# NVlabs/gbrl

Hardware: AMD Instinct MI355X
Metric: trees-fit/sec + predict rows/sec at batch=2^20, feat=128, depth=6, out=8 (higher is better)
Workload: dtype int32 fixed-point sums / f32 scores

## Files before the change

gbrl_amd/csrc/quantile.hip:

```cpp
#include "kernels.h"
#include "hooks.h"
#include "kernels_common.h"
#include "small_prep.h"

#include <algorithm>
#include <cstdint>
#include <cstdlib>

namespace gbrl {
namespace kern {

namespace {

constexpr int kMaxSplit = 4095;
constexpr int kClasses = 2 * (kMaxSplit + 1);

__global__ __launch_bounds__(256) void k_transpose_keys(const float *__restrict__ obs, int n, int F, uint32_t *__restrict__ kt) {
    __shared__ uint32_t tile[64][65];
    const int r0 = blockIdx.x * 64, f0 = blockIdx.y * 64;
    const int tx = threadIdx.x & 63, ty = threadIdx.x >> 6;
    for (int i = ty; i < 64; i += 4) {
        const int r = r0 + i, f = f0 + tx;
        tile[i][tx] = (r < n && f < F) ? float_to_key(obs[static_cast<size_t>(r) * F + f]) : 0xffffffffu;
    }
    __syncthreads();
    for (int i = ty; i < 64; i += 4) {
        const int f = f0 + i, r = r0 + tx;
        if (f < F && r < n) kt[static_cast<size_t>(f) * n + r] = tile[tx][i];
    }
}

__global__ __launch_bounds__(256) void k_transpose_keys_v4(const float *__restrict__ obs, int n, int F, uint32_t *__restrict__ kt) {
    __shared__ uint32_t tile[64][65];
    const int r0 = blockIdx.x * 64, f0 = blockIdx.y * 64;
    const int q = threadIdx.x & 15, p = threadIdx.x >> 4;
    float4 v[4];
#pragma unroll
    for (int i = 0; i < 4; ++i) {
        const int r = r0 + i * 16 + p, f = f0 + 4 * q;
        v[i] = (r < n && f < F) ? *reinterpret_cast<const float4 *>(obs + static_cast<size_t>(r) * F + f) : make_float4(0.f, 0.f, 0.f, 0.f);
    }
#pragma unroll
    for (int i = 0; i < 4; ++i) {
        uint32_t *t = &tile[i * 16 + p][4 * q];
        t[0] = float_to_key(v[i].x); t[1] = float_to_key(v[i].y); t[2] = float_to_key(v[i].z); t[3] = float_to_key(v[i].w);
    }
    __syncthreads();
#pragma unroll
    for (int i = 0; i < 4; ++i) {
        const int f = f0 + i * 16 + p, r = r0 + 4 * q;
        if (f < F && r < n) {
            const uint4 o = make_uint4(tile[4 * q][i * 16 + p], tile[4 * q + 1][i * 16 + p], tile[4 * q + 2][i * 16 + p], tile[4 * q + 3][i * 16 + p]);
            *reinterpret_cast<uint4 *>(kt + static_cast<size_t>(f) * n + r) = o;
        }
    }
}

__global__ __launch_bounds__(1024) void k_sample_splitters(const uint32_t *__restrict__ kt, int n, int S, int n_split,
                                                           uint32_t *__restrict__ splitters, uint32_t *__restrict__ splitters_bfs,
                                                           uint32_t *__restrict__ sample_out ) {
    extern __shared__ uint32_t s[];
    const int f = blockIdx.x;
    const uint32_t *col = kt + static_cast<size_t>(f) * n;
    if (n <= S) {
        for (int i = threadIdx.x; i < S; i += blockDim.x) s[i] = i < n ? col[i] : 0xffffffffu;
    } else {
        const double stride = static_cast<double>(n) / S;
        for (int i = threadIdx.x; i < S; i += blockDim.x) {
            const long long lo = static_cast<long long>(i * stride), hi = static_cast<long long>((i + 1) * stride);
            uint32_t h = (static_cast<uint32_t>(i) * 2654435761u) ^ (static_cast<uint32_t>(f) * 40503u + 0x9e3779b9u);
            h ^= h >> 15; h *= 2246822519u; h ^= h >> 13;
            const long long span = hi > lo ? hi - lo : 1;
            long long idx = lo + static_cast<long long>(h % static_cast<uint32_t>(span));
            if (idx >= n) idx = n - 1;
            s[i] = col[idx];
        }
    }
    __syncthreads();
    if (sample_out) {
        for (int i = threadIdx.x; i < S; i += blockDim.x) sample_out[static_cast<size_t>(f) * S + i] = s[i];
        return;
    }
    for (int k = 2; k <= S; k <<= 1) {
        for (int j = k >> 1; j > 0; j >>= 1) {
            for (int i = threadIdx.x; i < S; i += blockDim.x) {
                const int ixj = i ^ j;
                if (ixj > i) {
                    const uint32_t a = s[i], b = s[ixj];
                    const bool up = (i & k) == 0;
                    if ((a > b) == up) { s[i] = b; s[ixj] = a; }
                }
            }
            __syncthreads();
        }
    }
    const int step = S / (n_split + 1);
    for (int j = threadIdx.x; j < n_split; j += blockDim.x) splitters[static_cast<size_t>(f) * kMaxSplit + j] = s[(j + 1) * step - 1];
    int levels = 0;
    while ((1 << levels) < n_split + 1) ++levels;
    for (int i = threadIdx.x; i < n_split; i += blockDim.x) {
        const int L = 31 - __clz(i + 1), pp = i + 1 - (1 << L);
        const int q = ((2 * pp + 1) << (levels - 1 - L)) - 1;
        splitters_bfs[static_cast<size_t>(f) * kMaxSplit + i] = s[(q + 1) * step - 1];
    }
}

__global__ __launch_bounds__(1024) void k_sort_quantiles(const uint32_t *__restrict__ kt, int n, int S, const int64_t *__restrict__ cum, int B,
                                                         uint32_t *__restrict__ thr_keys, float *__restrict__ thr_floats, int F,
                                                         uint16_t *__restrict__ codes) {
    extern __shared__ uint32_t s[];
    sort_quantiles_body<false>(kt, n, S, cum, B, thr_keys, thr_floats, F, static_cast<int>(blockIdx.x), codes, s);
}

__global__ __launch_bounds__(1024) void k_union_splitters(const int64_t *__restrict__ uni, int SU, int n_split,
                                                          uint32_t *__restrict__ splitters, uint32_t *__restrict__ splitters_bfs) {
    extern __shared__ uint32_t s[];
    const int f = blockIdx.x;
    for (int i = threadIdx.x; i < SU; i += blockDim.x) s[i] = static_cast<uint32_t>(uni[static_cast<size_t>(f) * SU + i]);
    __syncthreads();
    for (int k = 2; k <= SU; k <<= 1) {
        for (int j = k >> 1; j > 0; j >>= 1) {
            for (int i = threadIdx.x; i < SU; i += blockDim.x) {
                const int ixj = i ^ j;
                if (ixj > i) {
                    const uint32_t a = s[i], b = s[ixj];
                    const bool up = (i & k) == 0;
                    if ((a > b) == up) { s[i] = b; s[ixj] = a; }
                }
            }
            __syncthreads();
        }
    }
    const int step = SU / (n_split + 1);
    for (int j = threadIdx.x; j < n_split; j += blockDim.x) splitters[static_cast<size_t>(f) * kMaxSplit + j] = s[(j + 1) * step - 1];
    int levels = 0;
    while ((1 << levels) < n_split + 1) ++levels;
    for (int i = threadIdx.x; i < n_split; i += blockDim.x) {
        const int L = 31 - __clz(i + 1), pp = i + 1 - (1 << L);
        const int q = ((2 * pp + 1) << (levels - 1 - L)) - 1;
        splitters_bfs[static_cast<size_t>(f) * kMaxSplit + i] = s[(q + 1) * step - 1];
    }
}
__global__ void k_place_sample(const uint32_t *__restrict__ samp, int F, int S, int rank, int SU, int64_t *__restrict__ uni) {
    const size_t i = static_cast<size_t>(blockIdx.x) * blockDim.x + threadIdx.x;
    if (i >= static_cast<size_t>(F) * S) return;
    const size_t f = i / S, j = i % S;
    uni[f * SU + static_cast<size_t>(rank) * S + j] = samp[i];
}
__global__ void k_counts_to_i64(const uint32_t *__restrict__ partial, int n_chunks, size_t fc, int64_t *__restrict__ out) {
    const size_t i = static_cast<size_t>(blockIdx.x) * blockDim.x + threadIdx.x;
    if (i >= fc) return;
    int64_t v = 0;
    for (int q = 0; q < n_chunks; ++q) v += partial[static_cast<size_t>(q) * fc + i];
    out[i] = v;
}
__global__ __launch_bounds__(256) void k_select_count(const uint32_t *__restrict__ lists, const uint32_t *__restrict__ tgt_off,
                                                      const uint32_t *__restrict__ tgt_len, const uint32_t *__restrict__ prefix,
                                                      int bit, int n_targets, int64_t *__restrict__ counts) {
    const int t = blockIdx.x * (blockDim.x / kWave) + (threadIdx.x / kWave);
    const int lane = threadIdx.x & (kWave - 1);
    if (t >= n_targets) return;
    const uint32_t off = tgt_off[t];
    uint32_t c = 0;
    if (off < 0xfffffffeu) {
        const uint32_t trial = prefix[t] | (1u << bit);
        const uint32_t *keys = lists + off;
        const uint32_t m = tgt_len[t];
        for (uint32_t i = lane; i < m; i += kWave) c += keys[i] < trial ? 1u : 0u;
        for (int o = kWave / 2; o > 0; o >>= 1) c += __shfl_xor(c, o, kWave);
    }
    if (lane == 0) counts[t] = c;
}
__global__ void k_select_update(uint32_t *__restrict__ prefix, const int64_t *__restrict__ counts, const uint32_t *__restrict__ tgt_off,
                                const uint32_t *__restrict__ tgt_rank, int bit, int n_targets, uint32_t *__restrict__ thr_keys) {
    const int t = blockIdx.x * blockDim.x + threadIdx.x;
    if (t >= n_targets) return;
    if (tgt_off[t] >= 0xfffffffeu) return;
    uint32_t p = prefix[t];
    if (counts[t] < static_cast<int64_t>(tgt_rank[t])) p |= (1u << bit);
    prefix[t] = p;
    if (bit == 0) thr_keys[t] = p;
}

__device__ __forceinline__ int classify(const uint32_t *e, int levels, uint32_t key) {
    int i = 0;
    uint32_t last_ge = 0;
    bool went_left = false;
    for (int l = 0; l < levels; ++l) {
        const uint32_t v = e[i];
        const bool lt = v < key;
        if (!lt) { last_ge = v; went_left = true; }
        i = 2 * i + 1 + (lt ? 1 : 0);
    }
    const int j = i - ((1 << levels) - 1);
    return 2 * j + ((went_left && last_ge == key) ? 1 : 0);
}
constexpr int KQ = 8;
__device__ __forceinline__ void classifyN(const uint32_t *e, int levels, const uint32_t (&key)[KQ], int (&cls)[KQ]) {
    int i[KQ];
    uint32_t ge[KQ];
    bool wl[KQ];
#pragma unroll
    for (int q = 0; q < KQ; ++q) { i[q] = 0; ge[q] = 0; wl[q] = false; }
    for (int l = 0; l < levels; ++l) {
#pragma unroll
        for (int q = 0; q < KQ; ++q) {
            const uint32_t v = e[i[q]];
            const bool lt = v < key[q];
            if (!lt) { ge[q] = v; wl[q] = true; }
            i[q] = 2 * i[q] + 1 + (lt ? 1 : 0);
        }
    }
#pragma unroll
    for (int q = 0; q < KQ; ++q) cls[q] = 2 * (i[q] - ((1 << levels) - 1)) + ((wl[q] && ge[q] == key[q]) ? 1 : 0);
}

constexpr int kCountThreads = 512;
__global__ __launch_bounds__(kCountThreads) void k_class_count(const uint32_t *__restrict__ kt, int n, int n_split,
                                                               const uint32_t *__restrict__ splitters, int chunk,
                                                               uint32_t *__restrict__ partial ) {
    __shared__ uint32_t sp[kMaxSplit + 1];
    __shared__ uint32_t cnt[kClasses];
    const int f = blockIdx.y;
    for (int i = threadIdx.x; i < n_split; i += kCountThreads) sp[i] = splitters[static_cast<size_t>(f) * kMaxSplit + i];
    for (int i = threadIdx.x; i < kClasses; i += kCountThreads) cnt[i] = 0;
    __syncthreads();
    const uint32_t *col = kt + static_cast<size_t>(f) * n;
    const int lo = blockIdx.x * chunk, hi = min(n, lo + chunk);
    int levels = 0;
    while ((1 << levels) < n_split + 1) ++levels;
    int i = lo + threadIdx.x;
    for (; i + (KQ - 1) * kCountThreads < hi; i += KQ * kCountThreads) {
        uint32_t k[KQ];
#pragma unroll
        for (int q = 0; q < KQ; ++q) k[q] = col[i + q * kCountThreads];
        int cls[KQ];
        classifyN(sp, levels, k, cls);
#pragma unroll
        for (int q = 0; q < KQ; ++q) atomicAdd(&cnt[cls[q]], 1u);
    }
    for (; i < hi; i += kCountThreads) atomicAdd(&cnt[classify(sp, levels, col[i])], 1u);
    __syncthreads();
    uint32_t *dst = partial + (static_cast<size_t>(blockIdx.x) * gridDim.y + f) * kClasses;
    for (int c = threadIdx.x; c < kClasses; c += kCountThreads) dst[c] = cnt[c];
}

__global__ __launch_bounds__(1024) void k_targets(const uint32_t *__restrict__ partial, int n_chunks, int F,
                                                  const int64_t *__restrict__ global_counts ,
                                                  const uint32_t *__restrict__ splitters, const int64_t *__restrict__ cum, int B,
                                                  uint32_t *__restrict__ class_off ,
                                                  uint32_t *__restrict__ tgt_off ,
                                                  uint32_t *__restrict__ tgt_len, uint32_t *__restrict__ tgt_rank,
                                                  uint32_t *__restrict__ thr_keys ,
                                                  uint32_t *__restrict__ alloc , uint32_t max_elems,
                                                  uint32_t *__restrict__ overflow) {
    __shared__ uint32_t pre[kClasses];
    __shared__ int32_t tcls[1024];
    const int f = blockIdx.x;
    uint32_t *coff = class_off + static_cast<size_t>(f) * kClasses;
    __shared__ uint32_t loc_cnt[kClasses];
    for (int c = threadIdx.x; c < kClasses; c += blockDim.x) {
        uint32_t v = 0;
        for (int q = 0; q < n_chunks; ++q) v += partial[(static_cast<size_t>(q) * F + f) * kClasses + c];
        loc_cnt[c] = v;
        pre[c] = global_counts ? static_cast<uint32_t>(global_counts[static_cast<size_t>(f) * kClasses + c]) : v;
    }
    __syncthreads();
    {
        const int base = threadIdx.x * 8;
        uint32_t loc[8], run = 0;
        for (int q = 0; q < 8; ++q) { run += pre[base + q]; loc[q] = run; }
        __shared__ uint32_t tot[1024];
        tot[threadIdx.x] = run;
        __syncthreads();
        for (int o = 1; o < 1024; o <<= 1) {
            const uint32_t v = threadIdx.x >= o ? tot[threadIdx.x - o] : 0;
            __syncthreads();
            tot[threadIdx.x] += v;
            __syncthreads();
        }
        const uint32_t off = threadIdx.x ? tot[threadIdx.x - 1] : 0;
        for (int q = 0; q < 8; ++q) pre[base + q] = loc[q] + off;
        __syncthreads();
    }
    for (int k0 = 0; k0 < B; k0 += 1024) {
        const int k = k0 + threadIdx.x;
        int c = -1;
        uint32_t want = 0, before = 0;
        if (k < B) {
            want = static_cast<uint32_t>(cum[k]);
            int lo = 0, hi = kClasses - 1;
            while (lo < hi) {
                const int mid = (lo + hi) >> 1;
                if (pre[mid] < want) lo = mid + 1; else hi = mid;
            }
            c = lo;
            before = c ? pre[c - 1] : 0;
        }
        tcls[threadIdx.x] = c;
        __syncthreads();
        if (k < B) {
            const size_t t = static_cast<size_t>(f) * B + k;
            tgt_rank[t] = want - before;
            if (c & 1) {
                thr_keys[t] = splitters[static_cast<size_t>(f) * kMaxSplit + (c >> 1)];
                tgt_off[t] = 0xffffffffu;
                tgt_len[t] = 0;
            } else {
                const bool first = (threadIdx.x == 0) ? (coff[c] == 0xffffffffu) : (tcls[threadIdx.x - 1] != c);
                const uint32_t len = loc_cnt[c];
                if (first) {
                    const uint32_t off = atomicAdd(&alloc[0], len);
                    if (off + len > max_elems || off + len < off) { atomicExch(overflow, 1u); coff[c] = 0xfffffffeu; }
                    else coff[c] = off;
                }
                tgt_len[t] = len;
            }
        }
        __syncthreads();
        if (k < B && !(c & 1)) tgt_off[static_cast<size_t>(f) * B + k] = coff[c];
        __syncthreads();
    }
}

__global__ __launch_bounds__(kCountThreads) void k_extract(const uint32_t *__restrict__ kt, int n, int n_split,
                                                           const uint32_t *__restrict__ splitters, int chunk,
                                                           const uint32_t *__restrict__ class_off,
                                                           const uint32_t *__restrict__ partial, uint32_t *__restrict__ out) {
    __shared__ uint32_t sp[kMaxSplit + 1];
    __shared__ uint32_t cur[kClasses];
    const int f = blockIdx.y, F = gridDim.y;
    for (int i = threadIdx.x; i < n_split; i += kCountThreads) sp[i] = splitters[static_cast<size_t>(f) * kMaxSplit + i];
    {
        constexpr int PER = kClasses / kCountThreads;
        uint32_t off[PER];
#pragma unroll
        for (int u = 0; u < PER; ++u) off[u] = class_off[static_cast<size_t>(f) * kClasses + threadIdx.x + u * kCountThreads];
        for (unsigned q = 0; q < blockIdx.x; ++q) {
            uint32_t add[PER];
#pragma unroll
            for (int u = 0; u < PER; ++u) add[u] = partial[(static_cast<size_t>(q) * F + f) * kClasses + threadIdx.x + u * kCountThreads];
#pragma unroll
            for (int u = 0; u < PER; ++u) off[u] += add[u];
        }
#pragma unroll
        for (int u = 0; u < PER; ++u) {
            const uint32_t base = class_off[static_cast<size_t>(f) * kClasses + threadIdx.x + u * kCountThreads];
            cur[threadIdx.x + u * kCountThreads] = base < 0xfffffffeu ? off[u] : 0xffffffffu;
        }
    }
    __syncthreads();
    const uint32_t *col = kt + static_cast<size_t>(f) * n;
    const int lo = blockIdx.x * chunk, hi = min(n, lo + chunk);
    int levels = 0;
    while ((1 << levels) < n_split + 1) ++levels;
    int i = lo + threadIdx.x;
    for (; i + (KQ - 1) * kCountThreads < hi; i += KQ * kCountThreads) {
        uint32_t k[KQ];
#pragma unroll
        for (int q = 0; q < KQ; ++q) k[q] = col[i + q * kCountThreads];
        int cls[KQ];
        classifyN(sp, levels, k, cls);
#pragma unroll
        for (int q = 0; q < KQ; ++q)
            if (cur[cls[q]] != 0xffffffffu) out[atomicAdd(&cur[cls[q]], 1u)] = k[q];
    }
    for (; i < hi; i += kCountThreads) {
        const uint32_t key = col[i];
        const int cls = classify(sp, levels, key);
        if (cur[cls] != 0xffffffffu) out[atomicAdd(&cur[cls], 1u)] = key;
    }
}

__global__ __launch_bounds__(256) void k_select(const uint32_t *__restrict__ lists, const uint32_t *__restrict__ tgt_off,
                                                const uint32_t *__restrict__ tgt_len, const uint32_t *__restrict__ tgt_rank,
                                                int n_targets, uint32_t *__restrict__ thr_keys) {
    const int t = blockIdx.x * (blockDim.x / kWave) + (threadIdx.x / kWave);
    const int lane = threadIdx.x & (kWave - 1);
    if (t >= n_targets) return;
    const uint32_t off = tgt_off[t];
    if (off >= 0xfffffffeu) return;
    const uint32_t *keys = lists + off;
    const uint32_t m = tgt_len[t], r = tgt_rank[t];
    uint32_t p = 0;
    constexpr int R = 16;
    if (m <= kWave * R) {
        uint32_t k[R];
#pragma unroll
        for (int q = 0; q < R; ++q) k[q] = (lane + q * kWave) < m ? keys[lane + q * kWave] : 0xffffffffu;
        for (int bit = 31; bit >= 0; --bit) {
            const uint32_t trial = p | (1u << bit);
            uint32_t c = 0;
#pragma unroll
            for (int q = 0; q < R; ++q) c += k[q] < trial ? 1u : 0u;
            for (int o = kWave / 2; o > 0; o >>= 1) c += __shfl_xor(c, o, kWave);
            if (c < r) p = trial;
        }
    } else {
        for (int bit = 31; bit >= 0; --bit) {
            const uint32_t trial = p | (1u << bit);
            uint32_t c = 0;
            for (uint32_t i = lane; i < m; i += kWave) c += keys[i] < trial ? 1u : 0u;
            for (int o = kWave / 2; o > 0; o >>= 1) c += __shfl_xor(c, o, kWave);
            if (c < r) p = trial;
        }
    }
    if (lane == 0) thr_keys[t] = p;
}

constexpr int kGroup = 16;
constexpr int kBinTiles = 16;
__global__ __launch_bounds__(256) void k_bin_cols(const uint32_t *__restrict__ kt, int n, int F, const uint32_t *__restrict__ thr,
                                                  int B, int levels, int tiles_per_block, uint16_t *__restrict__ codes) {
    extern __shared__ uint32_t lds[];
    const int P = (1 << levels) - 1;
    uint32_t *t = lds;
    uint16_t *tile_buf = reinterpret_cast<uint16_t *>(lds + kGroup * P);
    const int g = blockIdx.y;
    for (int i = threadIdx.x; i < kGroup * P; i += 256) {
        const int fl = i / P, e = i % P, f = g * kGroup + fl;
        const int L = 31 - __clz(e + 1), pp = e + 1 - (1 << L);
        const int q = ((2 * pp + 1) << (levels - 1 - L)) - 1;
        t[i] = (f < F && q < B) ? thr[static_cast<size_t>(f) * B + q] : 0xffffffffu;
    }
    __syncthreads();
    for (int tile = 0; tile < tiles_per_block; ++tile) {
        const int r0 = (blockIdx.x * tiles_per_block + tile) * 256;
        if (r0 >= n) break;
        const int r = r0 + threadIdx.x;
        const int rr = r < n ? r : n - 1;
        uint32_t key[kGroup];
#pragma unroll
        for (int q = 0; q < kGroup; ++q) {
            const int f = g * kGroup + q;
            key[q] = kt[static_cast<size_t>(f < F ? f : F - 1) * n + rr];
        }
#pragma unroll
        for (int fl0 = 0; fl0 < kGroup; fl0 += 8) {
            int idx[8];
#pragma unroll
            for (int q = 0; q < 8; ++q) idx[q] = 0;
            for (int l = 0; l < levels; ++l) {
#pragma unroll
                for (int q = 0; q < 8; ++q) idx[q] = 2 * idx[q] + 1 + ((t[(fl0 + q) * P + idx[q]] < key[fl0 + q]) ? 1 : 0);
            }
#pragma unroll
            for (int q = 0; q < 8; ++q) {
                const int f = g * kGroup + fl0 + q;
                int code = idx[q] - P;
                if (code > B) code = B;
                tile_buf[threadIdx.x * kGroup + fl0 + q] = static_cast<uint16_t>((f < F && r < n) ? code : 0);
            }
        }
        __syncthreads();
        const int rows = min(256, n - r0);
        {
            uint4 *dst = reinterpret_cast<uint4 *>(codes + (static_cast<size_t>(g) * n + r0) * kGroup);
            const uint4 *src = reinterpret_cast<const uint4 *>(tile_buf);
            for (int i = threadIdx.x; i < rows * 2; i += 256) dst[i] = src[i];
        }
        __syncthreads();
    }
}

#define GBRL_BIN_STEP_L8_F0(U, T, K) \
    asm volatile("v_lshl_add_u32 %8, %0, 2, %24\n ds_read_b32 %8, %8 offset:0\n" \
                 "v_lshl_add_u32 %9, %1, 2, %24\n ds_read_b32 %9, %9 offset:1024\n" \
                 "v_lshl_add_u32 %10, %2, 2, %24\n ds_read_b32 %10, %10 offset:2048\n" \
                 "v_lshl_add_u32 %11, %3, 2, %24\n ds_read_b32 %11, %11 offset:3072\n" \
                 "v_lshl_add_u32 %12, %4, 2, %24\n ds_read_b32 %12, %12 offset:4096\n" \
                 "v_lshl_add_u32 %13, %5, 2, %24\n ds_read_b32 %13, %13 offset:5120\n" \
                 "v_lshl_add_u32 %14, %6, 2, %24\n ds_read_b32 %14, %14 offset:6144\n" \
                 "v_lshl_add_u32 %15, %7, 2, %24\n ds_read_b32 %15, %15 offset:7168\n" \
                 "s_waitcnt lgkmcnt(0)\n" \
                 "v_cmp_lt_u32 vcc, %8, %16\n v_addc_co_u32 %0, vcc, %0, %0, vcc\n" \
                 "v_cmp_lt_u32 vcc, %9, %17\n v_addc_co_u32 %1, vcc, %1, %1, vcc\n" \
                 "v_cmp_lt_u32 vcc, %10, %18\n v_addc_co_u32 %2, vcc, %2, %2, vcc\n" \
                 "v_cmp_lt_u32 vcc, %11, %19\n v_addc_co_u32 %3, vcc, %3, %3, vcc\n" \
                 "v_cmp_lt_u32 vcc, %12, %20\n v_addc_co_u32 %4, vcc, %4, %4, vcc\n" \
                 "v_cmp_lt_u32 vcc, %13, %21\n v_addc_co_u32 %5, vcc, %5, %5, vcc\n" \
                 "v_cmp_lt_u32 vcc, %14, %22\n v_addc_co_u32 %6, vcc, %6, %6, vcc\n" \
                 "v_cmp_lt_u32 vcc, %15, %23\n v_addc_co_u32 %7, vcc, %7, %7, vcc\n" \
                 : "+v"(U[0]), "+v"(U[1]), "+v"(U[2]), "+v"(U[3]), "+v"(U[4]), "+v"(U[5]), "+v"(U[6]), "+v"(U[7]), \
                   "=&v"(T[0]), "=&v"(T[1]), "=&v"(T[2]), "=&v"(T[3]), "=&v"(T[4]), "=&v"(T[5]), "=&v"(T[6]), "=&v"(T[7]) \
                 : "v"(K[0]), "v"(K[1]), "v"(K[2]), "v"(K[3]), "v"(K[4]), "v"(K[5]), "v"(K[6]), "v"(K[7]), "s"(lds_base) \
                 : "vcc", "memory")
#define GBRL_BIN_STEP_L8_F8(U, T, K) \
    asm volatile("v_lshl_add_u32 %8, %0, 2, %24\n ds_read_b32 %8, %8 offset:8192\n" \
                 "v_lshl_add_u32 %9, %1, 2, %24\n ds_read_b32 %9, %9 offset:9216\n" \
                 "v_lshl_add_u32 %10, %2, 2, %24\n ds_read_b32 %10, %10 offset:10240\n" \
                 "v_lshl_add_u32 %11, %3, 2, %24\n ds_read_b32 %11, %11 offset:11264\n" \
                 "v_lshl_add_u32 %12, %4, 2, %24\n ds_read_b32 %12, %12 offset:12288\n" \
                 "v_lshl_add_u32 %13, %5, 2, %24\n ds_read_b32 %13, %13 offset:13312\n" \
                 "v_lshl_add_u32 %14, %6, 2, %24\n ds_read_b32 %14, %14 offset:14336\n" \
                 "v_lshl_add_u32 %15, %7, 2, %24\n ds_read_b32 %15, %15 offset:15360\n" \
                 "s_waitcnt lgkmcnt(0)\n" \
                 "v_cmp_lt_u32 vcc, %8, %16\n v_addc_co_u32 %0, vcc, %0, %0, vcc\n" \
                 "v_cmp_lt_u32 vcc, %9, %17\n v_addc_co_u32 %1, vcc, %1, %1, vcc\n" \
                 "v_cmp_lt_u32 vcc, %10, %18\n v_addc_co_u32 %2, vcc, %2, %2, vcc\n" \
                 "v_cmp_lt_u32 vcc, %11, %19\n v_addc_co_u32 %3, vcc, %3, %3, vcc\n" \
                 "v_cmp_lt_u32 vcc, %12, %20\n v_addc_co_u32 %4, vcc, %4, %4, vcc\n" \
                 "v_cmp_lt_u32 vcc, %13, %21\n v_addc_co_u32 %5, vcc, %5, %5, vcc\n" \
                 "v_cmp_lt_u32 vcc, %14, %22\n v_addc_co_u32 %6, vcc, %6, %6, vcc\n" \
                 "v_cmp_lt_u32 vcc, %15, %23\n v_addc_co_u32 %7, vcc, %7, %7, vcc\n" \
                 : "+v"(U[0]), "+v"(U[1]), "+v"(U[2]), "+v"(U[3]), "+v"(U[4]), "+v"(U[5]), "+v"(U[6]), "+v"(U[7]), \
                   "=&v"(T[0]), "=&v"(T[1]), "=&v"(T[2]), "=&v"(T[3]), "=&v"(T[4]), "=&v"(T[5]), "=&v"(T[6]), "=&v"(T[7]) \
                 : "v"(K[0]), "v"(K[1]), "v"(K[2]), "v"(K[3]), "v"(K[4]), "v"(K[5]), "v"(K[6]), "v"(K[7]), "s"(lds_base) \
                 : "vcc", "memory")
#define GBRL_BIN_STEP_L9_F0(U, T, K) \
    asm volatile("v_lshl_add_u32 %8, %0, 2, %24\n ds_read_b32 %8, %8 offset:0\n" \
                 "v_lshl_add_u32 %9, %1, 2, %24\n ds_read_b32 %9, %9 offset:2048\n" \
                 "v_lshl_add_u32 %10, %2, 2, %24\n ds_read_b32 %10, %10 offset:4096\n" \
                 "v_lshl_add_u32 %11, %3, 2, %24\n ds_read_b32 %11, %11 offset:6144\n" \
                 "v_lshl_add_u32 %12, %4, 2, %24\n ds_read_b32 %12, %12 offset:8192\n" \
                 "v_lshl_add_u32 %13, %5, 2, %24\n ds_read_b32 %13, %13 offset:10240\n" \
                 "v_lshl_add_u32 %14, %6, 2, %24\n ds_read_b32 %14, %14 offset:12288\n" \
                 "v_lshl_add_u32 %15, %7, 2, %24\n ds_read_b32 %15, %15 offset:14336\n" \
                 "s_waitcnt lgkmcnt(0)\n" \
                 "v_cmp_lt_u32 vcc, %8, %16\n v_addc_co_u32 %0, vcc, %0, %0, vcc\n" \
                 "v_cmp_lt_u32 vcc, %9, %17\n v_addc_co_u32 %1, vcc, %1, %1, vcc\n" \
                 "v_cmp_lt_u32 vcc, %10, %18\n v_addc_co_u32 %2, vcc, %2, %2, vcc\n" \
                 "v_cmp_lt_u32 vcc, %11, %19\n v_addc_co_u32 %3, vcc, %3, %3, vcc\n" \
                 "v_cmp_lt_u32 vcc, %12, %20\n v_addc_co_u32 %4, vcc, %4, %4, vcc\n" \
                 "v_cmp_lt_u32 vcc, %13, %21\n v_addc_co_u32 %5, vcc, %5, %5, vcc\n" \
                 "v_cmp_lt_u32 vcc, %14, %22\n v_addc_co_u32 %6, vcc, %6, %6, vcc\n" \
                 "v_cmp_lt_u32 vcc, %15, %23\n v_addc_co_u32 %7, vcc, %7, %7, vcc\n" \
                 : "+v"(U[0]), "+v"(U[1]), "+v"(U[2]), "+v"(U[3]), "+v"(U[4]), "+v"(U[5]), "+v"(U[6]), "+v"(U[7]), \
                   "=&v"(T[0]), "=&v"(T[1]), "=&v"(T[2]), "=&v"(T[3]), "=&v"(T[4]), "=&v"(T[5]), "=&v"(T[6]), "=&v"(T[7]) \
                 : "v"(K[0]), "v"(K[1]), "v"(K[2]), "v"(K[3]), "v"(K[4]), "v"(K[5]), "v"(K[6]), "v"(K[7]), "s"(lds_base) \
                 : "vcc", "memory")
#define GBRL_BIN_STEP_L9_F8(U, T, K) \
    asm volatile("v_lshl_add_u32 %8, %0, 2, %24\n ds_read_b32 %8, %8 offset:16384\n" \
                 "v_lshl_add_u32 %9, %1, 2, %24\n ds_read_b32 %9, %9 offset:18432\n" \
                 "v_lshl_add_u32 %10, %2, 2, %24\n ds_read_b32 %10, %10 offset:20480\n" \
                 "v_lshl_add_u32 %11, %3, 2, %24\n ds_read_b32 %11, %11 offset:22528\n" \
                 "v_lshl_add_u32 %12, %4, 2, %24\n ds_read_b32 %12, %12 offset:24576\n" \
                 "v_lshl_add_u32 %13, %5, 2, %24\n ds_read_b32 %13, %13 offset:26624\n" \
                 "v_lshl_add_u32 %14, %6, 2, %24\n ds_read_b32 %14, %14 offset:28672\n" \
                 "v_lshl_add_u32 %15, %7, 2, %24\n ds_read_b32 %15, %15 offset:30720\n" \
                 "s_waitcnt lgkmcnt(0)\n" \
                 "v_cmp_lt_u32 vcc, %8, %16\n v_addc_co_u32 %0, vcc, %0, %0, vcc\n" \
                 "v_cmp_lt_u32 vcc, %9, %17\n v_addc_co_u32 %1, vcc, %1, %1, vcc\n" \
                 "v_cmp_lt_u32 vcc, %10, %18\n v_addc_co_u32 %2, vcc, %2, %2, vcc\n" \
                 "v_cmp_lt_u32 vcc, %11, %19\n v_addc_co_u32 %3, vcc, %3, %3, vcc\n" \
                 "v_cmp_lt_u32 vcc, %12, %20\n v_addc_co_u32 %4, vcc, %4, %4, vcc\n" \
                 "v_cmp_lt_u32 vcc, %13, %21\n v_addc_co_u32 %5, vcc, %5, %5, vcc\n" \
                 "v_cmp_lt_u32 vcc, %14, %22\n v_addc_co_u32 %6, vcc, %6, %6, vcc\n" \
                 "v_cmp_lt_u32 vcc, %15, %23\n v_addc_co_u32 %7, vcc, %7, %7, vcc\n" \
                 : "+v"(U[0]), "+v"(U[1]), "+v"(U[2]), "+v"(U[3]), "+v"(U[4]), "+v"(U[5]), "+v"(U[6]), "+v"(U[7]), \
                   "=&v"(T[0]), "=&v"(T[1]), "=&v"(T[2]), "=&v"(T[3]), "=&v"(T[4]), "=&v"(T[5]), "=&v"(T[6]), "=&v"(T[7]) \
                 : "v"(K[0]), "v"(K[1]), "v"(K[2]), "v"(K[3]), "v"(K[4]), "v"(K[5]), "v"(K[6]), "v"(K[7]), "s"(lds_base) \
                 : "vcc", "memory")

template <int LEVELS>
__global__ __launch_bounds__(256) void k_bin_cols_fast(const uint32_t *__restrict__ kt, int n, int F, const uint32_t *__restrict__ thr,
                                                       int B, int tiles_per_block, uint16_t *__restrict__ codes) {
    constexpr int S = 1 << LEVELS;
    extern __shared__ uint32_t lds[];
    uint32_t *t = lds;
    uint32_t *tile_buf = lds + kGroup * S;
    const uint32_t lds_base = static_cast<uint32_t>(reinterpret_cast<uintptr_t>(t));
    const int g = blockIdx.y;
    for (int i = threadIdx.x; i < kGroup * S; i += 256) {
        const int fl = i >> LEVELS, u = i & (S - 1), f = g * kGroup + fl;
        uint32_t v = 0xffffffffu;
        if (u > 0) {
            const int L = 31 - __clz(u), pp = u - (1 << L);
            const int q = ((2 * pp + 1) << (LEVELS - 1 - L)) - 1;
            if (f < F && q < B) v = thr[static_cast<size_t>(f) * B + q];
        }
        t[i] = v;
    }
    __syncthreads();
    for (int tile = 0; tile < tiles_per_block; ++tile) {
        const int r0 = (blockIdx.x * tiles_per_block + tile) * 256;
        if (r0 >= n) break;
        const int r = r0 + threadIdx.x;
        const int rr = r < n ? r : n - 1;
        uint32_t key[kGroup];
#pragma unroll
        for (int q = 0; q < kGroup; ++q) {
            const int f = g * kGroup + q;
            key[q] = kt[static_cast<size_t>(f < F ? f : F - 1) * n + rr];
        }
        uint32_t word[kGroup / 2];
#pragma unroll
        for (int half = 0; half < 2; ++half) {
            uint32_t u[8], tv[8], kk[8];
#pragma unroll
            for (int q = 0; q < 8; ++q) { u[q] = 1; kk[q] = key[half * 8 + q]; }
#pragma unroll
            for (int l = 0; l < LEVELS; ++l) {
                if constexpr (LEVELS == 8) { if (half == 0) { GBRL_BIN_STEP_L8_F0(u, tv, kk); } else { GBRL_BIN_STEP_L8_F8(u, tv, kk); } }
                else                       { if (half == 0) { GBRL_BIN_STEP_L9_F0(u, tv, kk); } else { GBRL_BIN_STEP_L9_F8(u, tv, kk); } }
            }
#pragma unroll
            for (int q = 0; q < 8; q += 2) {
                const int f0 = g * kGroup + half * 8 + q;
                uint32_t c0 = min(u[q] - S, static_cast<uint32_t>(B)), c1 = min(u[q + 1] - S, static_cast<uint32_t>(B));
                if (!(f0 < F && r < n)) c0 = 0;
                if (!(f0 + 1 < F && r < n)) c1 = 0;
                word[half * 4 + q / 2] = c0 | (c1 << 16);
            }
        }
        uint4 *row = reinterpret_cast<uint4 *>(tile_buf + threadIdx.x * 8);
        row[0] = make_uint4(word[0], word[1], word[2], word[3]);
        row[1] = make_uint4(word[4], word[5], word[6], word[7]);
        __syncthreads();
        const int rows = min(256, n - r0);
        {
            uint4 *dst = reinterpret_cast<uint4 *>(codes + (static_cast<size_t>(g) * n + r0) * kGroup);
            const uint4 *src = reinterpret_cast<const uint4 *>(tile_buf);
            for (int i = threadIdx.x; i < rows * 2; i += 256) dst[i] = src[i];
        }
        __syncthreads();
    }
}
#undef GBRL_BIN_STEP_L8_F0
#undef GBRL_BIN_STEP_L8_F8
#undef GBRL_BIN_STEP_L9_F0
#undef GBRL_BIN_STEP_L9_F8

__global__ void k_scatter_cat_codes_grouped(const uint16_t *__restrict__ cat_codes, int n, int Fc, int F,
                                            uint16_t *__restrict__ codes) {
    const size_t i = static_cast<size_t>(blockIdx.x) * blockDim.x + threadIdx.x;
    if (i >= static_cast<size_t>(n) * Fc) return;
    const size_t r = i / Fc;
    const int slot = F + static_cast<int>(i % Fc);
    codes[(static_cast<size_t>(slot / kGroup) * n + r) * kGroup + (slot % kGroup)] = cat_codes[i];
}

}

void transpose_keys(const float *obs, int n, int F, uint32_t *kt, hipStream_t s) {
    dim3 grid((n + 63) / 64, (F + 63) / 64);
    const bool plain = [] { const char *e = hooks::raw(hooks::TRANSPOSE_PLAIN); return e && e[0] == '1'; }();
    if ((F & 3) == 0 && (n & 3) == 0 && !plain && (reinterpret_cast<uintptr_t>(obs) & 15) == 0 && (reinterpret_cast<uintptr_t>(kt) & 15) == 0)
        hipLaunchKernelGGL(k_transpose_keys_v4, grid, dim3(256), 0, s, obs, n, F, kt);
    else
        hipLaunchKernelGGL(k_transpose_keys, grid, dim3(256), 0, s, obs, n, F, kt);
}

QuantilePlan quantile_plan(int n) {
    QuantilePlan p;
    int S = 64;
    while (S < n && S < 4096) S <<= 1;
    p.sample = S;
    p.n_split = S - 1 < kMaxSplit ? S - 1 : kMaxSplit;
    p.n_chunks = n >= (1 << 18) ? 8 : (n >= (1 << 15) ? 2 : 1);
    p.chunk = (n + p.n_chunks - 1) / p.n_chunks;
    return p;
}

void sample_splitters(const uint32_t *kt, int n, int F, const QuantilePlan &p, uint32_t *splitters, uint32_t *splitters_bfs, hipStream_t s) {
    static PerDeviceOnce attr;
    if (attr.first()) { (void)hipFuncSetAttribute(reinterpret_cast<const void *>(k_sample_splitters), hipFuncAttributeMaxDynamicSharedMemorySize, 64 * 1024 + 1024); }
    hipLaunchKernelGGL(k_sample_splitters, dim3(F), dim3(1024), p.sample * sizeof(uint32_t), s, kt, n, p.sample, p.n_split, splitters, splitters_bfs,
                       static_cast<uint32_t *>(nullptr));
}

void sample_only(const uint32_t *kt, int n, int F, int S, uint32_t *sample_out, hipStream_t s) {
    static PerDeviceOnce attr;
    if (attr.first()) { (void)hipFuncSetAttribute(reinterpret_cast<const void *>(k_sample_splitters), hipFuncAttributeMaxDynamicSharedMemorySize, 64 * 1024 + 1024); }
    hipLaunchKernelGGL(k_sample_splitters, dim3(F), dim3(1024), S * sizeof(uint32_t), s, kt, n, S, S - 1, static_cast<uint32_t *>(nullptr),
                       static_cast<uint32_t *>(nullptr), sample_out);
}
void place_sample(const uint32_t *samp, int F, int S, int rank, int SU, int64_t *uni, hipStream_t s) {
    const size_t tot = static_cast<size_t>(F) * S;
    hipLaunchKernelGGL(k_place_sample, dim3((tot + 255) / 256), dim3(256), 0, s, samp, F, S, rank, SU, uni);
}
void union_splitters(const int64_t *uni, int F, int SU, int n_split, uint32_t *splitters, uint32_t *splitters_bfs, hipStream_t s) {
    static PerDeviceOnce attr;
    if (attr.first()) { (void)hipFuncSetAttribute(reinterpret_cast<const void *>(k_union_splitters), hipFuncAttributeMaxDynamicSharedMemorySize, 160 * 1024); }
    hipLaunchKernelGGL(k_union_splitters, dim3(F), dim3(1024), SU * sizeof(uint32_t), s, uni, SU, n_split, splitters, splitters_bfs);
}
void counts_to_i64(const uint32_t *partial, int n_chunks, size_t fc, int64_t *out, hipStream_t s) {
    hipLaunchKernelGGL(k_counts_to_i64, dim3((fc + 255) / 256), dim3(256), 0, s, partial, n_chunks, fc, out);
}
void select_count(const uint32_t *lists, const uint32_t *tgt_off, const uint32_t *tgt_len, const uint32_t *prefix, int bit, int n_targets,
                  int64_t *counts, hipStream_t s) {
    hipLaunchKernelGGL(k_select_count, dim3((n_targets + 3) / 4), dim3(256), 0, s, lists, tgt_off, tgt_len, prefix, bit, n_targets, counts);
}
void select_update(uint32_t *prefix, const int64_t *counts, const uint32_t *tgt_off, const uint32_t *tgt_rank, int bit, int n_targets,
                   uint32_t *thr_keys, hipStream_t s) {
    hipLaunchKernelGGL(k_select_update, dim3((n_targets + 255) / 256), dim3(256), 0, s, prefix, counts, tgt_off, tgt_rank, bit, n_targets, thr_keys);
}

void class_count(const uint32_t *kt, int n, int F, const QuantilePlan &p, const uint32_t *splitters, uint32_t *partial, hipStream_t s) {
    hipLaunchKernelGGL(k_class_count, dim3(p.n_chunks, F), dim3(kCountThreads), 0, s, kt, n, p.n_split, splitters, p.chunk, partial);
}

void quantile_targets(const uint32_t *partial, const int64_t *global_counts, const uint32_t *splitters, const int64_t *cum, int F, int B,
                      const QuantilePlan &p, uint32_t *class_off, uint32_t *tgt_off, uint32_t *tgt_len, uint32_t *tgt_rank,
                      uint32_t *thr_keys, uint32_t *alloc, uint32_t max_elems, uint32_t *overflow, hipStream_t s) {
    hipLaunchKernelGGL(k_targets, dim3(F), dim3(1024), 0, s, partial, p.n_chunks, F, global_counts, splitters, cum, B, class_off, tgt_off,
                       tgt_len, tgt_rank, thr_keys, alloc, max_elems, overflow);
}

void quantile_extract(const uint32_t *kt, int n, int F, const QuantilePlan &p, const uint32_t *splitters, const uint32_t *class_off,
                      const uint32_t *partial, uint32_t *out, hipStream_t s) {
    hipLaunchKernelGGL(k_extract, dim3(p.n_chunks, F), dim3(kCountThreads), 0, s, kt, n, p.n_split, splitters, p.chunk, class_off,
                       partial, out);
}

void quantile_select(const uint32_t *lists, const uint32_t *tgt_off, const uint32_t *tgt_len, const uint32_t *tgt_rank, int n_targets,
                     uint32_t *thr_keys, hipStream_t s) {
    hipLaunchKernelGGL(k_select, dim3((n_targets + 3) / 4), dim3(256), 0, s, lists, tgt_off, tgt_len, tgt_rank, n_targets, thr_keys);
}

int sort_quantiles_max_rows() { return 4096; }
bool sort_quantiles_fits(int n, int B) { int S = 256; while (S < n) S <<= 1; return n <= sort_quantiles_max_rows() && (static_cast<size_t>(S) + B) * sizeof(uint32_t) <= 64 * 1024; }
void sort_quantiles(const uint32_t *kt, int n, int F, const int64_t *cum, int B, uint32_t *thr_keys, float *thr_floats, hipStream_t s, uint16_t *codes) {
    int S = 256;
    while (S < n) S <<= 1;
    static PerDeviceOnce attr;
    if (attr.first()) { (void)hipFuncSetAttribute(reinterpret_cast<const void *>(k_sort_quantiles), hipFuncAttributeMaxDynamicSharedMemorySize, 64 * 1024); }
    const int blocks = codes ? ((F + kCodeGroup - 1) / kCodeGroup) * kCodeGroup : F;
    hipLaunchKernelGGL(k_sort_quantiles, dim3(blocks), dim3(S / 4), (static_cast<size_t>(S) + B) * sizeof(uint32_t), s, kt, n, S, cum, B, thr_keys, thr_floats, F, codes);
}

void bin_cols(const uint32_t *kt, int n, int F, const uint32_t *thr_keys, int B, uint16_t *codes, hipStream_t s) {
    int levels = 1;
    while ((1 << levels) - 1 < B) ++levels;
    const size_t lds = static_cast<size_t>(kGroup) * ((1 << levels) - 1) * sizeof(uint32_t) + 256 * kGroup * sizeof(uint16_t);
    static PerDeviceOnce attr;
    if (attr.first()) { (void)hipFuncSetAttribute(reinterpret_cast<const void *>(k_bin_cols), hipFuncAttributeMaxDynamicSharedMemorySize, 160 * 1024); }
    const int groups = (F + kGroup - 1) / kGroup;
    const long long tiles = (static_cast<long long>(n) + 255) / 256;
    int tpb = static_cast<int>(std::min<long long>(kBinTiles, std::max<long long>(1, tiles * groups / 1024)));
    dim3 grid(static_cast<unsigned>((tiles + tpb - 1) / tpb), groups);
    const bool plain = [] { const char *e = hooks::raw(hooks::BIN_PLAIN); return e && e[0] == '1'; }();
    if (!plain && (levels == 8 || levels == 9)) {
        const size_t lds_fast = static_cast<size_t>(kGroup) * (1u << levels) * sizeof(uint32_t) + 256 * kGroup * sizeof(uint16_t);
        static PerDeviceOnce attr_fast;
        if (attr_fast.first()) {
            (void)hipFuncSetAttribute(reinterpret_cast<const void *>(k_bin_cols_fast<8>), hipFuncAttributeMaxDynamicSharedMemorySize, 64 * 1024);
            (void)hipFuncSetAttribute(reinterpret_cast<const void *>(k_bin_cols_fast<9>), hipFuncAttributeMaxDynamicSharedMemorySize, 64 * 1024);
        }
        if (levels == 8) hipLaunchKernelGGL(k_bin_cols_fast<8>, grid, dim3(256), lds_fast, s, kt, n, F, thr_keys, B, tpb, codes);
        else hipLaunchKernelGGL(k_bin_cols_fast<9>, grid, dim3(256), lds_fast, s, kt, n, F, thr_keys, B, tpb, codes);
        return;
    }
    hipLaunchKernelGGL(k_bin_cols, grid, dim3(256), lds, s, kt, n, F, thr_keys, B, levels, tpb, codes);
}

void scatter_cat_codes_grouped(const uint16_t *cat_codes, int n, int Fc, int F, uint16_t *codes, hipStream_t s) {
    const size_t tot = static_cast<size_t>(n) * Fc;
    hipLaunchKernelGGL(k_scatter_cat_codes_grouped, dim3((tot + 255) / 256), dim3(256), 0, s, cat_codes, n, Fc, F, codes);
}

}
}
```

Measured before the change: 538.0.

## Double-buffer key loads and replace block barriers with wave barriers in binning

Restructures the grouped binning kernel's tile loop so the next tile's keys load into a second register set while the current tile is binned. The workgroup-wide __syncthreads calls around the LDS staging buffer become wavefront fences plus wave barriers, because each wave now copies only the rows it wrote itself. This aims to hide global-load latency and drop block-level sync stalls, at the cost of more registers and a few redundant loads at the tail.

```diff
diff --git a/gbrl_amd/csrc/quantile.hip b/gbrl_amd/csrc/quantile.hip
--- a/gbrl_amd/csrc/quantile.hip
+++ b/gbrl_amd/csrc/quantile.hip
@@ -572,17 +572,21 @@
         t[i] = v;
     }
     __syncthreads();
-    for (int tile = 0; tile < tiles_per_block; ++tile) {
-        const int r0 = (blockIdx.x * tiles_per_block + tile) * 256;
-        if (r0 >= n) break;
-        const int r = r0 + threadIdx.x;
+    const int lane = threadIdx.x & 63, wave = threadIdx.x >> 6;
+    const int tile0 = blockIdx.x * tiles_per_block;
+    const int n_tiles = min(tiles_per_block, (n + 255) / 256 - tile0);
+    auto load_keys = [&](int r0, uint32_t (&key)[kGroup]) __attribute__((always_inline)) {
+        const int r = r0 + static_cast<int>(threadIdx.x);
         const int rr = r < n ? r : n - 1;
-        uint32_t key[kGroup];
 #pragma unroll
         for (int q = 0; q < kGroup; ++q) {
             const int f = g * kGroup + q;
             key[q] = kt[static_cast<size_t>(f < F ? f : F - 1) * n + rr];
         }
+    };
+    auto bin_tile = [&](const uint32_t (&key)[kGroup], int tile) __attribute__((always_inline)) {
+        const int r0 = (tile0 + tile) * 256;
+        const int r = r0 + threadIdx.x;
         uint32_t word[kGroup / 2];
 #pragma unroll
         for (int half = 0; half < 2; ++half) {
@@ -606,14 +610,28 @@
         uint4 *row = reinterpret_cast<uint4 *>(tile_buf + threadIdx.x * 8);
         row[0] = make_uint4(word[0], word[1], word[2], word[3]);
         row[1] = make_uint4(word[4], word[5], word[6], word[7]);
-        __syncthreads();
+        __builtin_amdgcn_fence(__ATOMIC_RELEASE, "wavefront");
+        __builtin_amdgcn_wave_barrier();
         const int rows = min(256, n - r0);
         {
             uint4 *dst = reinterpret_cast<uint4 *>(codes + (static_cast<size_t>(g) * n + r0) * kGroup);
             const uint4 *src = reinterpret_cast<const uint4 *>(tile_buf);
-            for (int i = threadIdx.x; i < rows * 2; i += 256) dst[i] = src[i];
-        }
-        __syncthreads();
+#pragma unroll
+            for (int h = 0; h < 2; ++h) {
+                const int c = wave * 128 + h * 64 + lane;
+                if (c < rows * 2) dst[c] = src[c];
+            }
+        }
+        __builtin_amdgcn_fence(__ATOMIC_RELEASE, "wavefront");
+        __builtin_amdgcn_wave_barrier();
+    };
+    uint32_t ka[kGroup], kb[kGroup];
+    load_keys(tile0 * 256, ka);
+    for (int tile = 0; tile < n_tiles; tile += 2) {
+        load_keys((tile0 + min(tile + 1, n_tiles - 1)) * 256, kb);
+        bin_tile(ka, tile);
+        load_keys((tile0 + min(tile + 2, n_tiles - 1)) * 256, ka);
+        if (tile + 1 < n_tiles) bin_tile(kb, tile + 1);
     }
 }
 #undef GBRL_BIN_STEP_L8_F0
```

Measured after the change: 542.0 (median of 6 runs). No clear change (+0.7%).
